# python-lz4/python-lz4

Measured on AMD Instinct MI355X. Metric: GiB/s uncompressed, device-resident, 64 KiB blocks (decompress; compress), higher is better.
Workload: dtype u8; 1 GPU; config 2: decompress 1M x 64 KiB blocks, device-resident, LZ4_compress_default input; blocks_per_gpu=1048576, block_size=65536, parallelism=shard1

## Files before the change

### python-lz4_amd/csrc/lz4m_decompress.hip

```cpp
#include "lz4m_common.h"
#include "lz4m_rows.h"
#include "lz4m_worker.h"
#include "../../include/lz4m.h"

#include <stdlib.h>
#include <string.h>

#include <atomic>
#include <mutex>

namespace lz4m {

constexpr int64_t kCoopMin = 64;

enum CopyKind : int { kNone = 0, kLiteral = 1, kMatch = 2 };

struct Copy {
    int kind;
    int64_t dpos;
    int64_t arg;
    int64_t len;
};

struct Lane {
// ... 747 lines not shown
                __builtin_amdgcn_fence(__ATOMIC_SEQ_CST, "workgroup");
                coop_copy_literal<SOLO>(d + op, s + q, lit, lane);
                __builtin_amdgcn_fence(__ATOMIC_SEQ_CST, "workgroup");
                coop_copy_match(d + opm, off, ml, lane);
                __builtin_amdgcn_fence(__ATOMIC_SEQ_CST, "workgroup");
                op = opm + ml;
                ip = qe;
                base = (op > kHistKeep ? op - kHistKeep : 0) & ~15;
                for (int32_t c = base + 16 * (int32_t)lane; c < op; c += 16 * kWave)
                    lds_st16(OB + (c - base), ld16(d + c));
                F = op;
                continue;
            }
            const bool act = (int)lane < nseq;
            const int32_t tk = act ? myseq : 0;
            const u32x4 w = HLD(IN + tk);
            const CoopSeq q = coop_parse(IN, tk, w);
            const int32_t lit = q.lit, off = q.off, ml = q.ml, adv = q.adv;
            const int32_t len = act ? lit + ml : 0;
            const int32_t o = op + wave_incl_sum(len) - len;
            const int32_t sabs = ib + myseq;
            const bool lit_ok = q.litx ? ib + q.litpos + lit <= iend - 32 && o + lit <= oend - 32
                                       : sabs + 1 <= iend - 17;
            const bool in_dict = DICT && off > o + lit && off <= o + lit + dlen && off >= 16 && o + lit - off + ml <= 0;
            const bool ok_nofit = act && q.simple && lit_ok && (!q.mlx || sabs + adv <= iend - 4) && off >= 1 &&
                                  (off <= o + lit || in_dict) && o + len < oend - 64;
            const bool ok = ok_nofit && o + len <= base + kHistW;
            const uint64_t bad = __ballot(act) & ~__ballot(ok);
            const int use = bad ? __builtin_ctzll(bad) : nseq;
            const bool fit_only = bad && ((__ballot(ok_nofit) >> use) & 1ull);
            if (use == 0 && !(fit_only && !fit_cut && op - base > kHistKeep)) break;
            fit_cut = fit_only;
            if (use == 0) continue;
            const bool u = (int)lane < use;
            const int32_t m = o + lit;
            const bool far = u && m - off < base;
            u32x4 pre = u32x4{0, 0, 0, 0};
            if (far) pre = ld16(d + (m - off) + (DICT && m - off < 0 ? ddelta : 0));
            if (u && lit > 0) {
                if (lit <= 12) {
                    HPUT(OB + (o - base), window_shift1(w), lit);
                } else {
                    for (int32_t i = 0; i < lit; i += 16)
                        HPUT(OB + (o - base + i), HLD(IN + q.litpos + i), lit - i);
                }
            }
            lds_wait();
            const int32_t src_end = m - off + (off < ml ? off : ml);
            const int32_t mend = m + ml;
            uint64_t pend = __ballot(u);
            while (pend) {
                const int32_t E = __builtin_amdgcn_readlane(m, __builtin_ctzll(pend));
                const bool mine = (pend >> lane) & 1ull;
                int32_t x = __builtin_amdgcn_update_dpp(-1, mine ? mend : -1, 0x138, 0xF, 0xF, false);
                x = max(x, __builtin_amdgcn_update_dpp(-1, x, 0x111, 0xF, 0xF, false));
                x = max(x, __builtin_amdgcn_update_dpp(-1, x, 0x112, 0xF, 0xF, false));
                x = max(x, __builtin_amdgcn_update_dpp(-1, x, 0x114, 0xF, 0xF, false));
                x = max(x, __builtin_amdgcn_update_dpp(-1, x, 0x118, 0xF, 0xF, false));
                x = max(x, __builtin_amdgcn_update_dpp(-1, x, 0x142, 0xA, 0xF, false));
                x = max(x, __builtin_amdgcn_update_dpp(-1, x, 0x143, 0xC, 0xF, false));
                const bool ready = mine && (src_end <= E || x <= m - off);
                if (ready) {
                    const int32_t s0 = m - off;
                    if (off >= 16) {
                        for (int32_t i = 0; i < ml; i += 16) {
                            const int32_t sp = s0 + i;
                            const u32x4 v = (i == 0 && far)   ? pre
                                            : sp >= base          ? HLD(OB + (sp - base))
                                                                  : ld16(d + sp + (DICT && sp < 0 ? ddelta : 0));
                            HPUT(OB + (m - base + i), v, ml - i);
                        }
                    } else {
                        const u32x4 pat = period_pattern(HLD(OB + (s0 - base)), (uint32_t)off);
                        const int32_t step = 16 - (16 % off);
                        for (int32_t i = 0; i < ml; i += step) HPUT(OB + (m - base + i), pat, ml - i);
                    }
                }
                lds_wait();
                pend &= ~__ballot(ready);
            }
            op = __builtin_amdgcn_readlane(o + len, use - 1);
            ip = ib + __builtin_amdgcn_readlane(myseq + adv, use - 1);
            for (int32_t c = F + 16 * (int32_t)lane; c + 16 <= op; c += 16 * kWave)
                st16(d + c, lds_ld16(OB + (c - base)));
            F += (op - F) & ~15;
            if (use < nseq && !fit_only) break;
        }
        if (SOLO) LZ4M_WTS(ts, 4);
        for (int32_t c = F + 16 * (int32_t)lane; c < op; c += 16 * kWave)
            gbl_put(d + c, lds_ld16(OB + (c - base)), op - c);
        __builtin_amdgcn_fence(__ATOMIC_SEQ_CST, "workgroup");
        if (SOLO) LZ4M_WTS(ts, 5);
        const int32_t r = coop_finish<DICT, SOLO>(s, d, iend, oend, ip, op, fast, lane, dlen, d + ddelta);
        if (SOLO) LZ4M_WTS(ts, 6);
        if (lane == 0) status[b] = r;
        if (SOLO && lane == 0) solo_r = r;
    }
    if constexpr (SOLO) {
        __syncthreads();
        LZ4M_WTS(ts, 2);
        const int32_t r = solo_r;
        if (solo_out != nullptr && r > 0 && solo_lit < 0) {
            const uint8_t* d0 = dst + dst_off[0];
            constexpr int32_t kStep = 16 * 256, kChunk = 16 * kStep;
            lds_u8* bounce = (lds_u8*)const_cast<uint8_t*>(solo_src);
            for (int32_t c0 = 0; c0 < r; c0 += kChunk) {
                const int32_t m = r - c0 < kChunk ? r - c0 : kChunk;
                for (int32_t base0 = 0; base0 < m; base0 += kSoloU * kStep) {
                    u32x4 v[kSoloU];
#pragma unroll
                    for (int u = 0; u < kSoloU; ++u) {
                        const int32_t p = base0 + u * kStep + 16 * (int32_t)threadIdx.x;
                        v[u] = p + 16 <= m ? ld16(d0 + c0 + p) : ld16_guarded(d0 + c0 + p, m - p);
                    }
#pragma unroll
                    for (int u = 0; u < kSoloU; ++u) {
                        const int32_t p = base0 + u * kStep + 16 * (int32_t)threadIdx.x;
                        if (p < m) lds_st16(bounce + p, v[u]);
                    }
                }
                __syncthreads();
                for (int32_t p = 16 * (int32_t)threadIdx.x; p < m; p += kStep) {
                    const u32x4 v = lds_ld16(bounce + p);
                    if (p + 16 <= m) {
                        st16(solo_out + c0 + p, v);
                    } else {
                        put_exact(solo_out + c0 + p, v, (uint32_t)(m - p));
                    }
                }
                __syncthreads();
            }
        }
        if (solo_done != nullptr) {
            __builtin_amdgcn_fence(__ATOMIC_RELEASE, "");
            __syncthreads();
            LZ4M_WTS(ts, 3);
            if (threadIdx.x == 0) __hip_atomic_store(solo_done, 1, __ATOMIC_RELEASE, __HIP_MEMORY_SCOPE_SYSTEM);
        }
    }
#undef HPUT
#undef HLD
}

template <bool DICT, bool SOLO = false>
__global__ __launch_bounds__(256, 4) void hist_decompress_kernel(const uint8_t* __restrict__ src,
                                                                 const int64_t* __restrict__ src_off,
                                                                 const int32_t* __restrict__ src_len, uint8_t* dst,
                                                                 const int64_t* __restrict__ dst_off,
                                                                 const int32_t* __restrict__ dst_cap,
                                                                 int32_t* __restrict__ status, int64_t n,
                                                                 const int32_t* __restrict__ dict_len, int64_t ddelta,
                                                                 uint8_t* solo_out, int32_t* solo_done) {
    hist_decompress_body<DICT, SOLO>(src, src_off, src_len, dst, dst_off, dst_cap, status, n, dict_len, ddelta,
                                     solo_out, solo_done);
}

__global__ __launch_bounds__(256) void decompress_worker(Mailbox* mb, uint8_t* hd, uint8_t* dbuf, uint64_t idle,
                                                        uint64_t life) {
    __shared__ uint32_t cmd[8];
    __shared__ int64_t zero_off;
    uint64_t birth = 0;
    uint32_t last = worker_init(mb, cmd, birth);
    if (threadIdx.x == 0) zero_off = 0;
    for (;;) {
        if (worker_next(mb, last, idle, birth, life, cmd) == 0) break;
        const int32_t rec_off = (int32_t)cmd[1];
        CallMeta* rec = reinterpret_cast<CallMeta*>(hd + rec_off);
        const int32_t* len_cap = reinterpret_cast<const int32_t*>(cmd + 2);
        hist_decompress_body<false, true>(hd, &zero_off, len_cap, dbuf, &zero_off, len_cap + 1, &rec->result,
                                          (int64_t)1, nullptr, (int64_t)0, hd + rec_off + kCallMeta, &rec->done);
    }
}

__device__ __forceinline__ void chain_decode(const uint8_t* __restrict__ src, const int64_t* __restrict__ src_off,
                                             const int32_t* __restrict__ src_len,
                                             const uint8_t* __restrict__ raw_flag, uint8_t* dst,
                                             int32_t* __restrict__ status, int64_t n, int32_t max_block,
                                             uint32_t lane) {
    int64_t running = 0;
    for (int64_t b = 0; b < n; ++b) {
        const int64_t len = src_len[b];
        const uint8_t* s = src + src_off[b];
        uint8_t* d = dst + running;
        if (raw_flag[b]) {
            wave_copy_wild(d, s, len, len, len, lane);
            __builtin_amdgcn_fence(__ATOMIC_SEQ_CST, "workgroup");
            if (lane == 0) status[b] = (int32_t)len;
            running += len;
            continue;
        }
        Lane L;
        L.live = false;
        L.result = -1;
        if (lane == 0) {
            L.src = s;
            L.dst = d;
            L.iend = len;
            L.oend = max_block;
            L.ip = 0;
            L.op = 0;
            L.dict_len = running < 65536 ? running : 65536;
            L.dict_end = d;
            if (L.iend <= 0) {
                L.result = -1;
            } else {
                L.fast = L.oend >= 64;
                L.live = true;
            }
        }
        while (__any(L.live)) {
            Copy lc{kNone, 0, 0, 0}, mc{kNone, 0, 0, 0};
            if (L.live) decode_step<true>(L, lc, mc);
            const uint64_t pend = __ballot(lc.kind != kNone || mc.kind != kNone);
            if (pend == 0) continue;
            __builtin_amdgcn_fence(__ATOMIC_SEQ_CST, "workgroup");
            uint8_t* dd = readlane_ptr(L.dst, 0);
            const int64_t oend = readlane64(L.oend, 0);
            if (__builtin_amdgcn_readlane(lc.kind, 0) != kNone) {
                const uint8_t* ss = readlane_ptr(L.src, 0);
                const int64_t iend = readlane64(L.iend, 0);
                const int64_t dp = readlane64(lc.dpos, 0), sp = readlane64(lc.arg, 0), ln = readlane64(lc.len, 0);
                wave_copy_wild(dd + dp, ss + sp, ln, oend - dp, iend - sp, lane);
                __builtin_amdgcn_fence(__ATOMIC_SEQ_CST, "workgroup");
            }
            if (__builtin_amdgcn_readlane(mc.kind, 0) != kNone) {
                const int64_t dp = readlane64(mc.dpos, 0), off = readlane64(mc.arg, 0), ln = readlane64(mc.len, 0);
                if (off < 0) {
                    if (lane == 0) dict_match(L, dp, -off, ln);
                } else {
                    wave_match(dd + dp, off, ln, oend - dp, lane);
                }
                __builtin_amdgcn_fence(__ATOMIC_SEQ_CST, "workgroup");
            }
        }
        const int32_t r = __builtin_amdgcn_readlane(L.result, 0);
        if (lane == 0) status[b] = r;
        if (r < 0) {
            for (int64_t k = b + 1 + lane; k < n; k += kWave) status[k] = -1;
            return;
        }
        running += r;
    }
}

__global__ __launch_bounds__(64) void decompress_chain_kernel(const uint8_t* __restrict__ src,
                                                              const int64_t* __restrict__ src_off,
                                                              const int32_t* __restrict__ src_len,
                                                              const uint8_t* __restrict__ raw_flag, uint8_t* dst,
                                                              int32_t* __restrict__ status, int64_t n,
                                                              int32_t max_block) {
    chain_decode(src, src_off, src_len, raw_flag, dst, status, n, max_block, threadIdx.x);
}

__global__ __launch_bounds__(64) void decompress_chains_kernel(const uint8_t* __restrict__ src,
                                                               const int64_t* __restrict__ src_off,
                                                               const int32_t* __restrict__ src_len,
                                                               const uint8_t* __restrict__ raw_flag,
                                                               const int64_t* __restrict__ first,
                                                               const int32_t* __restrict__ count, uint8_t* dst,
                                                               const int64_t* __restrict__ dst_off,
                                                               const int32_t* __restrict__ max_block,
                                                               int32_t* __restrict__ status) {
    const int64_t c = blockIdx.x;
    const int64_t n = count[c];
    if (n <= 0) return;
    const int64_t f = first[c];
    chain_decode(src, src_off + f, src_len + f, raw_flag + f, dst + dst_off[c], status + f, n, max_block[c],
                 threadIdx.x);
}

}

using namespace lz4m;

namespace {

int current_device() {
    int dev = 0;
    (void)hipGetDevice(&dev);
    return dev >= 0 && dev < 64 ? dev : 0;
}

constexpr int kRowsMinBlocks = 32768;

enum Decoder { kAuto = 0, kHistDec = 3, kRowsDec = 4 };

int decoder_env() {
    static const int mode = [] {
        const char* e = getenv("LZ4M_DECODER");
        if (e == nullptr) return (int)kAuto;
        if (strcmp(e, "hist") == 0) return (int)kHistDec;
        if (strcmp(e, "rows") == 0) return (int)kRowsDec;
        return (int)kAuto;
    }();
    return mode;
}

}

extern "C" size_t lz4m_decompress_workspace_bytes(void) { return 64; }

extern "C" size_t lz4m_decompress_workspace_size(int64_t n, int64_t src_bytes) {
    if (n <= 0) return 64;
    const size_t lens = (size_t)(src_bytes > 0 ? src_bytes : 0) / 3 + 17 * (size_t)n + 64;
    return (lz4m_rows_fixed_bytes(n) + lens + 255) & ~(size_t)255;
}

extern "C" int lz4m_decompress_batch_sel(const uint8_t* d_src, const int64_t* d_src_off, const int32_t* d_src_len,
                                         uint8_t* d_dst, const int64_t* d_dst_off, const int32_t* d_dst_cap,
                                         int32_t* d_status, int64_t n, void* d_work, size_t work_bytes, int decoder,
                                         lz4m_stream_t stream) {
    if (n < 0 || !(decoder == kAuto || decoder == kHistDec || decoder == kRowsDec))
        return LZ4M_EINVAL;
    if (n == 0) return 0;
    hipStream_t st = (hipStream_t)stream;
    if (decoder == kAuto) decoder = decoder_env();
    if (d_work == nullptr || work_bytes < lz4m_decompress_workspace_bytes() || ((uintptr_t)d_work & 7) != 0)
        return LZ4M_EINVAL;
    const bool rows_fit = work_bytes >= lz4m_rows_fixed_bytes(n) + 64;
    if (decoder == kAuto) decoder = rows_fit && n >= kRowsMinBlocks ? kRowsDec : kHistDec;
    if (decoder != kHistDec && !rows_fit) decoder = kHistDec;
    if (decoder == kRowsDec) {
        int pg = 1, eg = 1;
        lz4m_rows_grids(n, &pg, &eg);
        const int rc = lz4m_rows_launch(d_src, d_src_off, d_src_len, d_dst, d_dst_off, d_dst_cap, n, d_work, work_bytes,
                                        pg, eg, st);
        if (rc != 0) return rc;
        const RowMeta* meta = reinterpret_cast<const RowMeta*>(static_cast<const uint8_t*>(d_work) + kRowsMeta);
        const int64_t grid = (n + 255) / 256;
        hipLaunchKernelGGL((decompress_kernel<false, true>), dim3((uint32_t)grid), dim3(256), 0, st, d_src, d_src_off,
                           d_src_len, d_dst, d_dst_off, d_dst_cap, nullptr, nullptr, nullptr, d_status, n, meta);
        return (int)hipGetLastError();
    }
    const int64_t grid = (n + 3) / 4;
    hipLaunchKernelGGL(hist_decompress_kernel<false>, dim3((uint32_t)(grid < 65536 ? grid : 65536)), dim3(256), 0, st,
                       d_src, d_src_off, d_src_len, d_dst, d_dst_off, d_dst_cap, d_status, n, nullptr, (int64_t)0, nullptr, nullptr);
    return (int)hipGetLastError();
}

extern "C" int lz4m_decompress_solo(const uint8_t* d_src, const int64_t* d_src_off, const int32_t* d_src_len,
                                    uint8_t* d_dst, const int64_t* d_dst_off, const int32_t* d_dst_cap,
                                    int32_t* d_status, int32_t src_len_host, uint8_t* h_out, int32_t* h_done,
                                    lz4m_stream_t stream) {
    if (src_len_host < 0 || src_len_host > kSoloIn - 64) return LZ4M_EINVAL;
    hipLaunchKernelGGL((hist_decompress_kernel<false, true>), dim3(1), dim3(256), 0, (hipStream_t)stream, d_src,
                       d_src_off, d_src_len, d_dst, d_dst_off, d_dst_cap, d_status, (int64_t)1, nullptr, (int64_t)0, h_out, h_done);
    return (int)hipGetLastError();
}

extern "C" int lz4m_worker_launch(int kind, Mailbox* mb, uint8_t* hd, uint8_t* dbuf, uint64_t idle_ticks,
                                  uint64_t life_ticks, hipStream_t stream) {
    if (kind == 1) return lz4m_compress_worker_launch(mb, hd, dbuf, idle_ticks, life_ticks, stream);
    if (kind != 0) return LZ4M_EINVAL;
    hipLaunchKernelGGL(decompress_worker, dim3(1), dim3(256), 0, stream, mb, hd, dbuf, idle_ticks, life_ticks);
    return (int)hipGetLastError();
}

extern "C" int lz4m_decompress_batch_ws(const uint8_t* d_src, const int64_t* d_src_off, const int32_t* d_src_len,
                                        uint8_t* d_dst, const int64_t* d_dst_off, const int32_t* d_dst_cap,
                                        int32_t* d_status, int64_t n, void* d_work, size_t work_bytes,
                                        lz4m_stream_t stream) {
    return lz4m_decompress_batch_sel(d_src, d_src_off, d_src_len, d_dst, d_dst_off, d_dst_cap, d_status, n, d_work,
                                     work_bytes, kAuto, stream);
}

extern "C" int lz4m_decompress_batch(const uint8_t* d_src, const int64_t* d_src_off, const int32_t* d_src_len,
                                     uint8_t* d_dst, const int64_t* d_dst_off, const int32_t* d_dst_cap,
                                     int32_t* d_status, int64_t n, lz4m_stream_t stream) {
    if (n < 0) return LZ4M_EINVAL;
    if (n == 0) return 0;
    const int64_t grid = (n + 3) / 4;
    hipLaunchKernelGGL(hist_decompress_kernel<false>, dim3((uint32_t)(grid < 65536 ? grid : 65536)), dim3(256), 0,
                       (hipStream_t)stream, d_src, d_src_off, d_src_len, d_dst, d_dst_off, d_dst_cap, d_status, n,
                       nullptr, (int64_t)0, nullptr, nullptr);
    return (int)hipGetLastError();
}

extern "C" int lz4m_decompress_batch_dict(const uint8_t* d_src, const int64_t* d_src_off, const int32_t* d_src_len,
                                          uint8_t* d_dst, const int64_t* d_dst_off, const int32_t* d_dst_cap,
                                          const uint8_t* d_dict, const int64_t* d_dict_off,
                                          const int32_t* d_dict_len, int32_t* d_status, int64_t n,
                                          lz4m_stream_t stream) {
    if (n < 0) return LZ4M_EINVAL;
    if (n == 0) return 0;
    const int64_t grid = (n + 255) / 256;
    hipLaunchKernelGGL(decompress_kernel<true>, dim3((uint32_t)grid), dim3(256), 0, (hipStream_t)stream, d_src,
                       d_src_off, d_src_len, d_dst, d_dst_off, d_dst_cap, d_dict, d_dict_off, d_dict_len, d_status,
                       n, nullptr);
    return (int)hipGetLastError();
}

extern "C" int lz4m_decompress_batch_prefix(const uint8_t* d_src, const int64_t* d_src_off, const int32_t* d_src_len,
                                            uint8_t* d_dst, const int64_t* d_dst_off, const int32_t* d_dst_cap,
                                            const uint8_t* d_dict_base, const int32_t* d_dict_len,
                                            int32_t* d_status, int64_t n, lz4m_stream_t stream) {
    if (n < 0 || (n > 0 && d_dict_base == nullptr)) return LZ4M_EINVAL;
    if (n == 0) return 0;
    const int64_t grid = (n + 3) / 4;
    const int64_t delta = (int64_t)((intptr_t)d_dict_base - (intptr_t)d_dst);
    hipLaunchKernelGGL(hist_decompress_kernel<true>, dim3((uint32_t)(grid < 65536 ? grid : 65536)), dim3(256), 0,
                       (hipStream_t)stream, d_src, d_src_off, d_src_len, d_dst, d_dst_off, d_dst_cap, d_status, n,
                       d_dict_len, delta, nullptr, nullptr);
    return (int)hipGetLastError();
}

extern "C" int lz4m_decompress_chain(const uint8_t* d_src, const int64_t* d_src_off, const int32_t* d_src_len,
                                     const uint8_t* d_raw_flag, uint8_t* d_dst, int32_t* d_status, int64_t n,
                                     int32_t max_block, lz4m_stream_t stream) {
    if (n < 0 || max_block < 0) return LZ4M_EINVAL;
    if (n == 0) return 0;
    hipLaunchKernelGGL(decompress_chain_kernel, dim3(1), dim3(64), 0, (hipStream_t)stream, d_src, d_src_off,
                       d_src_len, d_raw_flag, d_dst, d_status, n, max_block);
    return (int)hipGetLastError();
}


extern "C" int lz4m_decompress_chains(const uint8_t* d_src, const int64_t* d_src_off, const int32_t* d_src_len,
                                      const uint8_t* d_raw_flag, const int64_t* d_first, const int32_t* d_count,
                                      uint8_t* d_dst, const int64_t* d_dst_off, const int32_t* d_max_block,
                                      int32_t* d_status, int64_t n_chains, lz4m_stream_t stream) {
    if (n_chains < 0 || n_chains > 0x7FFFFFFF) return LZ4M_EINVAL;
    if (n_chains == 0) return 0;
    if (!d_first || !d_count || !d_dst_off || !d_max_block || !d_status) return LZ4M_EINVAL;
    hipLaunchKernelGGL(decompress_chains_kernel, dim3((uint32_t)n_chains), dim3(64), 0, (hipStream_t)stream, d_src,
                       d_src_off, d_src_len, d_raw_flag, d_first, d_count, d_dst, d_dst_off, d_max_block, d_status);
    return (int)hipGetLastError();
}
```

### python-lz4_amd/csrc/lz4m_rows.hip

```cpp
#include "lz4m_common.h"
#include "lz4m_rows.h"

namespace lz4m {
typedef __attribute__((address_space(3))) u32x4 lds_u32x4;

__device__ __forceinline__ void wait_vm0() { __builtin_amdgcn_s_waitcnt(0x0F70); }

__device__ __forceinline__ void row_incl_sum2(int32_t& a, int32_t& b) {
    a += __builtin_amdgcn_update_dpp(0, a, 0x111, 0xF, 0xF, false);
    b += __builtin_amdgcn_update_dpp(0, b, 0x111, 0xF, 0xF, false);
    a += __builtin_amdgcn_update_dpp(0, a, 0x112, 0xF, 0xF, false);
    b += __builtin_amdgcn_update_dpp(0, b, 0x112, 0xF, 0xF, false);
    a += __builtin_amdgcn_update_dpp(0, a, 0x114, 0xF, 0xF, false);
    b += __builtin_amdgcn_update_dpp(0, b, 0x114, 0xF, 0xF, false);
    a += __builtin_amdgcn_update_dpp(0, a, 0x118, 0xF, 0xF, false);
    b += __builtin_amdgcn_update_dpp(0, b, 0x118, 0xF, 0xF, false);
}
__device__ __forceinline__ int32_t row_last(int32_t v) { return __builtin_amdgcn_update_dpp(0, v, 0x15F, 0xF, 0xF, false); }
__device__ __forceinline__ int32_t row_first(int32_t v) { return __builtin_amdgcn_update_dpp(0, v, 0x150, 0xF, 0xF, false); }

__device__ __forceinline__ void row_excl_max2(int32_t a, int32_t b, int32_t& xa, int32_t& xb) {
    int32_t x = __builtin_amdgcn_update_dpp(0, a, 0x111, 0xF, 0xF, false);
    int32_t y = __builtin_amdgcn_update_dpp(0, b, 0x111, 0xF, 0xF, false);
    x = max(x, __builtin_amdgcn_update_dpp(0, x, 0x111, 0xF, 0xF, false));
// ... 72 lines not shown

__device__ __forceinline__ int64_t whole_literal_block(const uint8_t* s, int32_t iend, int32_t oend, uint8_t* d,
                                                       uint32_t lane) {
    typedef __attribute__((address_space(1))) const uint8_t gu8;
    const int32_t y = 16 * (int32_t)lane;
    const u32x4 v = y + 16 <= iend ? ld16(s + y) : ld16_guarded(s + y, iend - y);
    const uint32_t tok = (uint32_t)__builtin_amdgcn_readlane((int32_t)v.x, 0) & 0xFFu;
    int32_t first = 16;
    for (int b = 15; b >= 0; --b)
        if (byte_of(v, b) != 255u && (lane != 0 || b != 0)) first = b;
    const uint64_t nz = __ballot(first < 16 && y + first < iend);
    if ((tok >> 4) != 15u || nz == 0) return -1;
    const int fl = __builtin_ctzll(nz);
    const int32_t pe = 16 * fl + __builtin_amdgcn_readlane(first, fl);
    const uint32_t bt = (uint32_t)__builtin_amdgcn_readlane((int32_t)byte_of(v, first & 15), fl);
    const int64_t L = 15 + 255 * (int64_t)(pe - 1) + bt;
    const int32_t q = pe + 1;
    if (q > iend - 15 || q + L != (int64_t)iend || L > oend) return -1;
    const uint8_t* cs = (const uint8_t*)(gu8*)(s + q);
    const uint32_t Lf = (uint32_t)L & ~15u;
    for (uint32_t b = 0; b < Lf; b += 4096) {
        u32x4 w[4];
#pragma unroll
        for (int u = 0; u < 4; ++u) {
            const uint32_t p = b + 1024u * u + (uint32_t)y;
            if (p < Lf) w[u] = ld16(cs + p);
        }
#pragma unroll
        for (int u = 0; u < 4; ++u) {
            const uint32_t p = b + 1024u * u + (uint32_t)y;
            if (p < Lf) st16(d + p, w[u]);
        }
    }
    if ((uint32_t)L != Lf && lane == ((Lf >> 4) & 63u)) row_put(d + Lf, ld16_guarded(cs + Lf, (int32_t)L - (int32_t)Lf), (int32_t)L - (int32_t)Lf);
    return L;
}

__global__ __launch_bounds__(kPWG) void rows_parse_kernel(const uint8_t* __restrict__ src,
                                                         const int64_t* __restrict__ src_off,
                                                         const int32_t* __restrict__ src_len,
                                                         uint8_t* __restrict__ dst,
                                                         const int64_t* __restrict__ dst_off,
                                                         const int32_t* __restrict__ dst_cap, int64_t n,
                                                         RowMeta* __restrict__ meta, uint8_t* __restrict__ lens,
                                                         int64_t lens_cap, unsigned long long* __restrict__ ctr) {
    __shared__ __attribute__((aligned(kPW))) uint8_t wins[kPWG * kPW];
    __shared__ __attribute__((aligned(kPStage))) uint8_t stgs[kPWG * kPStage];
    const uint32_t lane = lane_id();
    lds_u8* W = (lds_u8*)(wins + threadIdx.x * kPW);
    const uint32_t Wa = (uint32_t)(uintptr_t)W;
    lds_u8* stg = (lds_u8*)(stgs + threadIdx.x * kPStage);
    const uint32_t Sa = (uint32_t)(uintptr_t)stg;
    const uint8_t* s = nullptr;
    int64_t idx = -1, loff = 0;
    int32_t iend = 0, oend = 0, ip = 0, op = 0, k = 0, kf = 0, wb = 0, sh = 0;
    u32x4 pf[4];
    bool live = false, need = false, more = true, pfv = false, stall = false;
    while (true) {
        if (more) {
            const uint64_t idle = __ballot(!live);
            if (idle != 0 && (uint32_t)__popcll(idle) >= 8u) {
                const int first = __builtin_ctzll(idle);
                const uint32_t cnt = (uint32_t)__popcll(idle);
                unsigned long long qb = 0;
                if ((int)lane == first) qb = atomicAdd(&ctr[0], (unsigned long long)cnt);
                qb = (unsigned long long)readlane64((int64_t)qb, first);
                if (qb + cnt >= (unsigned long long)n) more = false;
                int64_t wantb = 0;
                bool fresh = false;
                if (!live) {
                    const uint64_t below = lane == 0 ? 0 : (idle & (~0ull >> (64 - lane)));
                    idx = (int64_t)(qb + (unsigned long long)__popcll(below));
                    if (idx < n) {
                        const int64_t so = src_off[idx];
                        const int32_t il = src_len[idx];
                        sh = (int32_t)((uintptr_t)(src + so) & 63u);
                        if (so < sh) sh = 0;
                        s = src + so - sh;
                        iend = il + sh;
                        oend = dst_cap[idx];
                        ip = sh;
                        op = k = kf = 0;
                        wb = -4 * kPW;
                        pfv = false;
                        if (oend >= 64 && il > 0) {
                            const int32_t a = il / 3, b = oend / 4;
                            wantb = ((int64_t)(a < b ? a : b) + 1 + 15) & ~(int64_t)15;
                            fresh = true;
                        } else {
                            meta[idx] = RowMeta{0, 0, 0, 0, 0, 0};
                        }
                    }
                }
                int64_t incl = wantb;
#pragma unroll
                for (int dd = 1; dd < 64; dd <<= 1) {
                    const int64_t t = __shfl_up(incl, dd);
                    if ((int)lane >= dd) incl += t;
                }
                const int64_t total = readlane64(incl, 63);
                int64_t abase = 0;
                if (total > 0) {
                    if (lane == 0) abase = (int64_t)atomicAdd(&ctr[1], (unsigned long long)total);
                    abase = readlane64(abase, 0);
                }
                if (fresh) {
                    loff = abase + incl - wantb;
                    if (loff + wantb > lens_cap) {
                        meta[idx] = RowMeta{0, 0, 0, 0, 0, 0};
                    } else {
                        live = true;
                        need = true;
                    }
                }
            }
        }
        if (!__any(live)) {
            if (more) continue;
            break;
        }
        {
            const uint64_t R = __ballot(live && pfv && ip >= wb + 64);
            if (R) {
#pragma unroll
                for (int c = 0; c < 4; ++c) {
                    const int bb = 16 * c + (int)(lane >> 2);
                    const int32_t wbb = __builtin_amdgcn_ds_bpermute(bb << 2, wb);
                    if ((R >> bb) & 1ull) {
                        lds_u8* Wb = (lds_u8*)(wins + bb * kPW);
                        const int32_t h = (wbb >> 6) & 1;
                        lds_st16(Wb + 64 * h + 16 * (int32_t)(lane & 3), pf[c]);
                    }
                }
                if ((R >> lane) & 1ull) {
                    wb += 64;
                    pfv = false;
                }
            }
        }
        if (live && stall && !need && ip + 16 > wb + kPW) need = true;
        stall = false;
        bool wl = false;
        if (live && need) {
            need = false;
            if (ip + 32 > wb + kPW) {
                const int32_t nb = ip & ~63;
                u32x4 v0[4], v1[4];
                load64(s, nb, iend, v0);
                load64(s, nb + 64, iend, v1);
                ring_put(W, (nb >> 6) & 1, v0);
                ring_put(W, ((nb >> 6) + 1) & 1, v1);
                wb = nb;
                pfv = false;
            }
            bool good = true, slow = true;
            int32_t pe = 0;
            int64_t lit = 0, ml = 0;
            {
                const uint32_t x0 = __builtin_amdgcn_alignbyte(*(lds_vu32*)(size_t)(Wa | (((uint32_t)ip + 4u) & (kPW - 4))),
                                                               *(lds_vu32*)(size_t)(Wa | ((uint32_t)ip & (kPW - 4))), (uint32_t)ip);
                const uint32_t tok = x0 & 0xFFu;
                const int32_t l0 = (int32_t)(tok >> 4), mlc = (int32_t)(tok & 15u);
                int32_t q = 1, L = l0;
                bool g = true, sl = false;
                if (l0 == 15) {
                    if (ip + 1 >= iend - 15) {
                        g = false;
                    } else {
                        const int32_t e = (int32_t)((x0 >> 8) & 0xFFu);
                        q = 2;
                        L += e;
                        if (ip + 2 > iend - 15) g = false;
                        else if (e == 255) sl = true;
                        if (g && !sl && (op + L > oend - 32 || ip + q + L > iend - 32)) g = false;
                    }
                } else if (ip + 1 > iend - 17) {
                    g = false;
                }
                int32_t M = mlc, pq = 0;
                if (g && !sl) {
                    const int32_t po = q + L;
                    if (po + 3 > 32) {
                        sl = true;
                    } else {
                        const uint32_t ao = (uint32_t)(ip + po);
                        const uint32_t dw = __builtin_amdgcn_alignbyte(*(lds_vu32*)(size_t)(Wa | ((ao + 4u) & (kPW - 4))),
                                                                       *(lds_vu32*)(size_t)(Wa | (ao & (kPW - 4))), ao);
                        const int32_t off = (int32_t)(dw & 0xFFFFu);
                        pq = po + 2;
                        if (mlc == 15) {
                            const int32_t e2 = (int32_t)((dw >> 16) & 0xFFu);
                            ++pq;
                            M += e2;
                            if (ip + pq > iend - 4) g = false;
                            else if (e2 == 255) sl = true;
                        }
                        M += 4;
                        if (g && !sl && (off == 0 || off > op + L || op + L + M >= oend - 64)) g = false;
                    }
                }
                slow = sl;
                if (!sl) {
                    good = g;
                    pe = ip + pq;
                    lit = L;
                    ml = M;
                }
            }
            if (slow) {
#define PB(x) ((x) - wb < kPW ? (uint32_t)W[(x) & (kPW - 1)] : (uint32_t)s[(x)])
                good = true;
                const uint32_t tok = PB(ip);
                lit = tok >> 4;
                int32_t q = ip + 1;
                if (lit == 15) {
                    if (q >= iend - 15) {
                        good = false;
                    } else {
                        uint32_t b;
                        int32_t run = 0;
                        do {
                            b = PB(q);
                            ++q;
                            lit += b;
                            if (q > iend - 15) good = false;
                            if (++run >= kPRunCap && b == 255) {
                                good = false;
                                wl = k == 0;
                            }
                        } while (good && b == 255);
                        if (good && (op + lit > oend - 32 || q + lit > iend - 32)) good = false;
                    }
                } else if (q > iend - 17) {
                    good = false;
                }
                if (good) {
                    const int32_t po = q + (int32_t)lit;
                    const uint32_t off = PB(po) | (PB(po + 1) << 8);
                    pe = po + 2;
                    ml = tok & 15;
                    if (ml == 15) {
                        uint32_t b;
                        int32_t run = 0;
                        do {
                            b = PB(pe);
                            ++pe;
                            ml += b;
                            if (pe > iend - 4) good = false;
                            if (++run >= kPRunCap && b == 255) good = false;
                        } while (good && b == 255);
                    }
                    ml += 4;
                    if (good && (off == 0 || (int64_t)off > (int64_t)op + lit || (int64_t)op + lit + ml >= (int64_t)oend - 64))
                        good = false;
                }
#undef PB
            }
            if (good) {
                const int32_t adv = pe - ip;
                stg[k & (kPStage - 1)] = (uint8_t)(adv < 255 ? adv : 255);
                ip = pe;
                op += (int32_t)(lit + ml);
                ++k;
            } else {
                for (int32_t c = kf; c < k; c += 16) row_put(lens + loff + c, lds_ld16(stg + (c & (kPStage - 1))), k - c);
                meta[idx] = RowMeta{loff, k, ip - sh, op, 0, 0};
                live = false;
            }
        }
        for (uint64_t C = __ballot(wl); C != 0; C &= C - 1) {
            const int f = __builtin_ctzll(C);
            const int64_t fi = readlane64(idx, f);
            const int32_t fsh = __builtin_amdgcn_readlane(sh, f);
            const int64_t r = whole_literal_block(readlane_ptr(s, f) + fsh, __builtin_amdgcn_readlane(iend, f) - fsh,
                                                  __builtin_amdgcn_readlane(oend, f), dst + dst_off[fi], lane);
            if ((int)lane == f && r >= 0) meta[idx] = RowMeta{loff, 0, kRowsWholeLiteral, (int32_t)r, 0, 0};
        }
        if (live && k - kf >= kPStage / 2) {
            uint8_t* o = lens + loff + kf;
            st16(o, lds_ld16(stg + (kf & (kPStage - 1))));
            kf += kPStage / 2;
        }
        {
            const uint64_t Q = __ballot(live && !pfv && wb + kPW < iend);
            if (Q) {
                const uint64_t na = (uint64_t)(uintptr_t)(s + wb + kPW);
                const int32_t left = iend - (wb + kPW);
#pragma unroll
                for (int c = 0; c < 4; ++c) {
                    const int bb = 16 * c + (int)(lane >> 2);
                    const uint32_t lo = (uint32_t)__builtin_amdgcn_ds_bpermute(bb << 2, (int32_t)(uint32_t)na);
                    const uint32_t hi = (uint32_t)__builtin_amdgcn_ds_bpermute(bb << 2, (int32_t)(uint32_t)(na >> 32));
                    const int32_t lf = __builtin_amdgcn_ds_bpermute(bb << 2, left) - 16 * (int32_t)(lane & 3);
                    if ((Q >> bb) & 1ull) {
                        const uint8_t* q = readlane_safe_ptr(((uint64_t)hi << 32) | lo) + 16 * (lane & 3);
                        pf[c] = lf >= 16 ? ld16(q) : ld16_guarded(q, lf);
                    }
                }
                if ((Q >> lane) & 1ull) pfv = true;
            }
        }
        const int32_t thr = min(kPMinActive, (int)__popcll(__ballot(live)));
        const int32_t kfl = kf + kPStage - 1;
        auto peek = [&](int32_t& lit, int32_t& adv, int32_t& ml, int32_t& off, int32_t& oe) __attribute__((always_inline)) {
            const int32_t tok = (int32_t)*(lds_vu8*)(size_t)(Wa | ((uint32_t)ip & (kPW - 1)));
            lit = tok >> 4;
            const int32_t mlc = tok & 15;
            const int32_t ob = ip + 1 + lit;
            const uint32_t lo = *(lds_vu32*)(size_t)(Wa | ((uint32_t)ob & (kPW - 4)));
            const uint32_t hi = *(lds_vu32*)(size_t)(Wa | ((uint32_t)(ob + 4) & (kPW - 4)));
            const uint32_t dw = __builtin_amdgcn_alignbyte(hi, lo, (uint32_t)ob);
            const bool mlx = mlc == 15;
            off = (int32_t)(dw & 0xFFFFu);
            adv = 3 + lit + (int32_t)mlx;
            ml = mlc + 4 + (mlx ? (int32_t)((dw >> 16) & 0xFFu) : 0);
            oe = op + lit + ml;
        };
        {
            const int32_t lim = min(wb + kPW - 16, iend - 20);
            const int32_t oendm = oend - 64;
            bool go = live && !need && !stall;
            while (true) {
#pragma unroll
                for (int u = 0; u < kPSteps; ++u) {
                    int32_t lit, adv, ml, off, oe;
                    peek(lit, adv, ml, off, oe);
                    const bool take = go & (ip <= lim) & (k < kfl) & (lit <= 12) & (ml != 274) &
                                      ((uint32_t)(off - 1) < (uint32_t)(op + lit)) & (oe < oendm);
                    *(lds_vu8*)(size_t)(Sa | ((uint32_t)k & (kPStage - 1))) = (uint8_t)adv;
                    ip += take ? adv : 0;
                    op = take ? oe : op;
                    k += (int32_t)take;
                    go = take;
                }
                if ((int)__popcll(__ballot(go)) < max(thr, 1)) break;
            }
            if (live && !need && !stall && !go) {
                int32_t lit, adv, ml, off, oe;
                peek(lit, adv, ml, off, oe);
                const bool fast = (lit <= 12) & (ml != 274) & (ip <= iend - 20) & (off != 0) & (off <= op + lit) &
                                  (oe < oendm);
                stall = true;
                need = (ip + 16 <= wb + kPW) & (k < kfl) & !fast;
            }
        }
    }
}

constexpr int32_t kRowsH = 1280;
constexpr int32_t kRowsHS = kRowsH + 32;
constexpr int32_t kRowsRoom = 512;
constexpr int32_t kRowsKeep = kRowsH - kRowsRoom;
static_assert(kRowsKeep % 16 == 0 && kRowsKeep + kRowsRoom <= kRowsH && kRowsKeep + 16 <= 1024, "history split");

__device__ __forceinline__ void row_copy_literal(uint8_t* d, const uint8_t* s, int32_t len, int32_t jj) {
    for (int32_t pos = 16 * jj; pos < len; pos += 256) {
        const u32x4 v = len - pos >= 16 ? ld16(s + pos) : ld16_guarded(s + pos, len - pos);
        row_put(d + pos, v, len - pos);
    }
}

__device__ __forceinline__ void row_copy_match(uint8_t* d, int32_t off, int32_t len, int32_t jj) {
    if (off >= 16) {
        const int32_t w = off & ~15;
        for (int32_t b = 0; b < len; b += w) {
            const int32_t e = min(b + w, len);
            for (int32_t p0 = b + 16 * jj; p0 < e; p0 += 1024) {
                u32x4 v[4];
#pragma unroll
                for (int u = 0; u < 4; ++u)
                    if (p0 + 256 * u < e) v[u] = ld16(d + p0 + 256 * u - off);
#pragma unroll
                for (int u = 0; u < 4; ++u)
                    if (p0 + 256 * u < e) row_put(d + p0 + 256 * u, v[u], len - (p0 + 256 * u));
            }
            __builtin_amdgcn_fence(__ATOMIC_SEQ_CST, "workgroup");
        }
        return;
    }
    const u32x4 pat = period_pattern(ld16(d - off), (uint32_t)off);
    const int32_t step = 16 - (16 % off);
    for (int32_t pos = step * jj; pos < len; pos += step * 16) row_put(d + pos, pat, len - pos);
}


#define LDS_PUT(p, v, k) lds_put_al((p), (v), (k), MT)

#define ROFF(x) ((uint32_t)(x))

struct PSeq {
    int32_t t, lit, off, ml, o, dlt;
    int32_t opn, ipn;
    uint32_t fl;
};
constexpr uint32_t kFlU = 1, kFlFar = 2, kFlLate = 4, kFlLitHbm = 8, kFlEsc = 16;

struct FarSrc {
    u32x4 g0, g1;
};

__device__ __forceinline__ void parse_round(PSeq& P, int32_t jj, int32_t r, int32_t k0, int32_t nseq, int32_t ip,
                                            int32_t op, int32_t bnext, int32_t F, const uint8_t* s, const uint8_t* d,
                                            int32_t iend, int32_t dlt, int32_t t, u32x4 wa, u32x4 wb, lds_u32x4* XS,
                                            FarSrc& FS, int32_t& incsum) {
    const bool act = k0 + jj < nseq;
    const bool esc = dlt == 255;
    const bool wbok = t + 32 <= iend;
    const uint32_t tok = wa.x & 0xFFu;
    const int32_t lit0 = (int32_t)(tok >> 4);
    const bool litx = lit0 == 15;
    const int32_t lit = lit0 + (litx ? (int32_t)byte_of(wa, 1) : 0);
    const int32_t lp = litx ? 2 : 1;
    const int32_t po = lp + lit;
    const int32_t mlc = (int32_t)(tok & 15u);
    const uint32_t pq = (uint32_t)(po < 28 ? po : 28);
    const uint32_t dwo = dword32_tree(wa, wb, pq);
    const uint32_t bsh = po > 28 ? 8u : 0u;
    int32_t off = (int32_t)((dwo >> bsh) & 0xFFFFu);
    const int32_t e0 = (int32_t)((dwo >> (bsh + 16)) & 0xFFu);
    int32_t ml = mlc + (mlc == 15 ? e0 : 0);
    const bool slow = (po + 3 > 32) | ((mlc == 15) & (e0 == 255)) | ((po + 3 > 16) & !wbok);
    if (slow && act && !esc) {
        const uint8_t* q = s + t;
        off = (int32_t)q[po] | ((int32_t)q[po + 1] << 8);
        ml = mlc;
        if (ml == 15) {
            int32_t pe = po + 2;
            uint32_t b;
            do {
                b = q[pe];
                ++pe;
                ml += (int32_t)b;
            } while (b == 255 && pe < iend - t);
        }
    }
    ml += 4;
    const int32_t len = act && !esc ? lit + ml : 0;
    int32_t lsum = len;
    row_incl_sum2(lsum, incsum);
    const int32_t o = op + lsum - len;
    const int32_t mend = o + lit + ml;
    const bool ok = act & !esc & (mend <= bnext + kRowsH);
    const uint64_t nok = __ballot(!ok);
    int32_t use;
    bool u;
    if (nok == 0) {
        use = 16;
        u = true;
        P.opn = row_last(o + len);
        P.ipn = row_last(t + dlt);
    } else {
        const uint32_t rb = (uint32_t)(nok >> (16 * r)) & 0xFFFFu;
        use = rb ? __builtin_ctz(rb) : 16;
        u = jj < use;
        P.opn = op + row_last(row_incl_sum(u ? len : 0));
        P.ipn = ip + row_last(row_incl_sum(u ? dlt : 0));
    }
    const int32_t s0 = o + lit - off;
    const bool far = u & (s0 < bnext);
    const bool late = far & (s0 + 32 > F);
    const bool pf = far & !late;
    FS.g0 = ld16(d + ROFF(pf ? s0 : 0));
    FS.g1 = ld16(d + ROFF((pf & (ml > 16)) ? s0 + 16 : 0));
    const uint32_t sh = (uint32_t)lp;
    XS[0] = u32x4{__builtin_amdgcn_alignbyte(wa.y, wa.x, sh), __builtin_amdgcn_alignbyte(wa.z, wa.y, sh),
                 __builtin_amdgcn_alignbyte(wa.w, wa.z, sh), __builtin_amdgcn_alignbyte(wb.x, wa.w, sh)};
    XS[1] = u32x4{__builtin_amdgcn_alignbyte(wb.y, wb.x, sh), __builtin_amdgcn_alignbyte(wb.z, wb.y, sh),
                 __builtin_amdgcn_alignbyte(wb.w, wb.z, sh), __builtin_amdgcn_alignbyte(0u, wb.w, sh)};
    P.t = t + lp;
    P.lit = lit;
    P.off = off;
    P.ml = ml;
    P.o = o;
    P.dlt = dlt;
    P.fl = ((uint32_t)use << 8) | (u ? kFlU : 0u) | (far ? kFlFar : 0u) | (late ? kFlLate : 0u) | (esc ? kFlEsc : 0u) |
           ((u & (lp + lit > 16) & ((lp + lit > 32) | !wbok)) ? kFlLitHbm : 0u);
}

__device__ __forceinline__ int32_t cold_j16(int32_t jj) {
    int32_t v = 16 * jj;
    asm volatile("" : "+v"(v));
    return v;
}

__device__ __forceinline__ int32_t next_base(int32_t op, int32_t base) {
    return op - base > kRowsH - kRowsRoom ? ((op - kRowsKeep) & ~15) : base;
}

__device__ __forceinline__ void load_in(const uint8_t* s, int32_t t, int32_t iend, u32x4& a, u32x4& b) {
    const int32_t ta = t + 16 <= iend ? t : 0;
    const int32_t tb = t + 32 <= iend ? t + 16 : iend - 16;
    a = ld16(s + ROFF(ta));
    b = ld16(s + ROFF(tb));
}
__device__ __forceinline__ int32_t load_len(const uint8_t* dl, int32_t k, int32_t nseq) {
    return (int32_t)dl[ROFF(k < nseq ? k : nseq - 1)];
}


constexpr int kEWG = 256;
__global__ __launch_bounds__(kEWG) __attribute__((amdgpu_waves_per_eu(5, 8))) void rows_exec_kernel(const uint8_t* __restrict__ src,
                                                       const int64_t* __restrict__ src_off,
                                                       const int32_t* __restrict__ src_len, uint8_t* dst,
                                                       const int64_t* __restrict__ dst_off,
                                                       const RowMeta* __restrict__ meta,
                                                       const uint8_t* __restrict__ lens, int64_t n,
                                                       unsigned long long* __restrict__ ctr) {
    __shared__ __attribute__((aligned(16))) uint8_t hists[kEWG / 16 * kRowsHS];
    __shared__ __attribute__((aligned(16))) uint32_t mtab[kPutTab];
    __shared__ __attribute__((aligned(16))) uint32_t psel[16 * 8];
    __shared__ __attribute__((aligned(16))) u32x4 xsl[kEWG * 2];
    const uint32_t lane = threadIdx.x & 63u;
    const int32_t jj = (int32_t)(lane & 15), r = (int32_t)(lane >> 4);
    lds_u8* HB = (lds_u8*)(hists + (threadIdx.x >> 4) * kRowsHS);
    lds_put_table_init(mtab, threadIdx.x, kEWG);
    lds_cu32* MT = (lds_cu32*)mtab;
    period_sel_init(psel, threadIdx.x, kEWG);
    __syncthreads();
    lds_cu32* PS = (lds_cu32*)psel;
    lds_u32x4* XSL = (lds_u32x4*)(xsl + 2 * threadIdx.x);
    const uint8_t* s = nullptr;
    uint8_t* d = nullptr;
    const uint8_t* dl = nullptr;
    int32_t iend = 0, nseq = 0, k0 = 0, ip = 0, op = 0, base = 0, F = 0;
    bool have = false, sync = true;
    PSeq P, Q;
    FarSrc FS;
    int32_t incq = 0, lraw = 0;
    u32x4 na = u32x4{0, 0, 0, 0}, nb = na;
    while (true) {
        if (!have) {
            unsigned long long b = 0;
            if (jj == 0) b = atomicAdd(&ctr[2], 1ull);
            const uint32_t blo = (uint32_t)row_first((int32_t)(uint32_t)b);
            const uint32_t bhi = (uint32_t)row_first((int32_t)(uint32_t)(b >> 32));
            b = ((unsigned long long)bhi << 32) | blo;
            if (b >= (unsigned long long)n) break;
            const RowMeta mt = meta[b];
            if (mt.nseq == 0) continue;
            s = src + src_off[b];
            d = dst + dst_off[b];
            iend = src_len[b];
            dl = lens + mt.loff;
            nseq = mt.nseq;
            k0 = ip = op = base = F = 0;
            have = true;
            sync = true;
        }
        if (sync && k0 >= nseq) {
            for (int32_t c = F + cold_j16(jj); c < op; c += 256) row_put(d + c, lds_ld16(HB + (c - base)), op - c);
            have = false;
            continue;
        }
        if (sync) {
            const int32_t dc = load_len(dl, k0 + jj, nseq);
            const int32_t dq = load_len(dl, k0 + 16 + jj, nseq);
            lraw = load_len(dl, k0 + 32 + jj, nseq);
            int32_t incc = dc;
            incq = dq;
            row_incl_sum2(incc, incq);
            const int32_t tc = ip + incc - dc;
            u32x4 wa, wb;
            load_in(s, tc, iend, wa, wb);
            load_in(s, ip + row_last(incc) + incq - dq, iend, na, nb);
            int32_t dummy = 0;
            parse_round(P, jj, r, k0, nseq, ip, op, base, F, s, d, iend, dc, tc, wa, wb, XSL, FS, dummy);
            sync = false;
            if ((P.fl >> 8) != 0) wait_vm0();
        }
        if ((P.fl >> 8) == 0) {
            sync = true;
            int32_t L, q, ofs, qe, M;
            if (!(row_first((int32_t)P.fl) & kFlEsc)) {
                L = row_first(P.lit);
                q = row_first(P.t);
                ofs = row_first(P.off);
                M = row_first(P.ml);
                qe = q + L + 2 + (M >= 19 ? (M - 19) / 255 + 1 : 0);
            } else {
                const uint32_t tk = s[ip];
                L = (int32_t)(tk >> 4);
                q = ip + 1;
                if (L == 15) {
                    uint32_t b;
                    do {
                        b = s[q];
                        ++q;
                        L += (int32_t)b;
                    } while (b == 255 && q < iend);
                }
                ofs = (int32_t)s[q + L] | ((int32_t)s[q + L + 1] << 8);
                qe = q + L + 2;
                M = (int32_t)(tk & 15u);
                if (M == 15) {
                    uint32_t b;
                    do {
                        b = s[qe];
                        ++qe;
                        M += (int32_t)b;
                    } while (b == 255 && qe < iend);
                }
                M += 4;
            }
            for (int32_t c = F + cold_j16(jj); c < op; c += 256) row_put(d + c, lds_ld16(HB + (c - base)), op - c);
            row_copy_literal(d + op, s + q, L, jj);
            __builtin_amdgcn_fence(__ATOMIC_SEQ_CST, "workgroup");
            row_copy_match(d + op + L, ofs, M, jj);
            __builtin_amdgcn_fence(__ATOMIC_SEQ_CST, "workgroup");
            op += L + M;
            ip = qe;
            k0 += 1;
            base = (op > kRowsKeep ? op - kRowsKeep : 0) & ~15;
            for (int32_t c = base + cold_j16(jj); c < op; c += 256) lds_st16(HB + (c - base), ld16(d + c));
            F = op;
            continue;
        }
        {
            const bool u = (P.fl & kFlU) != 0;
            const int32_t lit = P.lit, o = P.o;
            if (u && lit > 0) LDS_PUT(HB + (o - base), XSL[0], lit);
            if (u && lit > 16) {
                if (!(P.fl & kFlLitHbm)) {
                    LDS_PUT(HB + (o - base + 16), XSL[1], lit - 16);
                } else {
                    for (int32_t i = 16; i < lit; i += 16) LDS_PUT(HB + (o - base + i), ld16(s + P.t + i), lit - i);
                }
            }
        }
        const bool ahead = (P.fl >> 8) == 16 && k0 + 16 < nseq;
        auto parse_ahead = [&]() __attribute__((always_inline)) {
            if (ahead) {
                const int32_t bq = next_base(P.opn, base);
                const int32_t dq = incq - __builtin_amdgcn_update_dpp(0, incq, 0x111, 0xF, 0xF, true);
                int32_t inc2 = lraw;
                parse_round(Q, jj, r, k0 + 16, nseq, P.ipn, P.opn, bq, F, s, d, iend, dq, P.ipn + incq - dq, na, nb, XSL, FS, inc2);
                incq = inc2;
                load_in(s, Q.ipn + incq - lraw, iend, na, nb);
                lraw = load_len(dl, k0 + 48 + jj, nseq);
            }
        };
        const bool u = (P.fl & kFlU) != 0;
        const int32_t lit = P.lit, off = P.off, ml = P.ml, o = P.o;
        const int32_t m = o + lit, mend = m + ml, s0 = m - off;
        const bool far = (P.fl & kFlFar) != 0, late = (P.fl & kFlLate) != 0;
        u32x4 g0 = FS.g0;
        const u32x4 g1 = FS.g1;
        if (__any(late)) {
            const u32x4 lv = ld16(d + ROFF(late ? s0 : 0));
            g0 = late ? lv : g0;
        }
        const int32_t se = s0 + (off < ml ? off : ml);
        const bool per = off < 16;
        constexpr uint64_t kRem16 = (0ull << 3) | (0ull << 6) | (1ull << 9) | (0ull << 12) | (1ull << 15) |
                                    (4ull << 18) | (2ull << 21) | (0ull << 24) | (7ull << 27) | (6ull << 30) |
                                    (5ull << 33) | (4ull << 36) | (3ull << 39) | (2ull << 42) | (1ull << 45);
        const int32_t stp = per ? 16 - (int32_t)((kRem16 >> (3u * ((uint32_t)off & 15u))) & 7u) : 16;
        bool pend = u;
        auto copy_match = [&]() __attribute__((always_inline)) {
            const u32x4 l0 = lds_ld16a(HB + (s0 >= base ? s0 - base : 0));
            u32x4 v0 = far ? g0 : l0;
            if (per) v0 = period_perm(l0, PS + 8 * off);
            LDS_PUT(HB + (m - base), v0, ml);
            if (ml > stp) {
                for (int32_t i = stp; i < ml; i += stp) {
                    u32x4 v = v0;
                    if (!per) {
                        const int32_t sp = s0 + i;
                        v = lds_ld16a(HB + (sp >= base ? sp - base : 0));
                        const bool pc1 = (i == 16) & far & !late;
                        if (sp < base && pc1) v = g1;
                        const bool hb = (sp < base) & !pc1;
                        if (__any(hb)) {
                            const u32x4 x = ld16(d + ROFF(hb ? sp : 0));
                            v = hb ? x : v;
                        }
                    }
                    LDS_PUT(HB + (m - base + i), v, ml - i);
                }
            }
        };
        while (__any(pend)) {
            int32_t x1, y1;
            row_excl_max2(pend ? mend + 1 : 0, pend ? 0x3FFFFFFF - m : 0, x1, y1);
            const bool ready = pend & ((x1 <= s0 + 1) | (y1 <= 0x3FFFFFFF - se));
            if (ready) copy_match();
            pend = pend && !ready;
        }
        parse_ahead();
        const int32_t opn = P.opn;
        {
            const int32_t fe = opn & ~127;
            for (int32_t c = F + 16 * jj; c + 16 <= fe; c += 256) st16(d + ROFF(c), lds_ld16(HB + (c - base)));
            if (fe > F) F += (fe - F) & ~15;
        }
        op = opn;
        ip = P.ipn;
        k0 += (int32_t)(P.fl >> 8);
        const int32_t nbse = next_base(op, base);
        if (nbse != base) {
            for (int32_t c0 = 0; c0 < op - nbse; c0 += 1024) {
                u32x4 v[4];
#pragma unroll
                for (int g = 0; g < 4; ++g) v[g] = lds_ld16(HB + (nbse - base) + c0 + 256 * g + 16 * jj);
#pragma unroll
                for (int g = 0; g < 4; ++g) lds_st16(HB + c0 + 256 * g + 16 * jj, v[g]);
            }
            base = nbse;
        }
        if (ahead) {
            P = Q;
        } else {
            sync = true;
        }
    }
}

}

using namespace lz4m;


extern "C" size_t lz4m_rows_fixed_bytes(int64_t n) { return kRowsMeta + (size_t)n * sizeof(RowMeta); }

extern "C" int lz4m_rows_launch(const uint8_t* d_src, const int64_t* d_src_off, const int32_t* d_src_len,
                                uint8_t* d_dst, const int64_t* d_dst_off, const int32_t* d_dst_cap, int64_t n,
                                void* d_work, size_t work_bytes, int parse_grid, int exec_grid, hipStream_t stream) {
    const size_t fixed = lz4m_rows_fixed_bytes(n);
    if (work_bytes < fixed) return LZ4M_ROWS_ENOSPACE;
    unsigned long long* ctr = static_cast<unsigned long long*>(d_work);
    RowMeta* meta = reinterpret_cast<RowMeta*>(static_cast<uint8_t*>(d_work) + kRowsMeta);
    uint8_t* lens = static_cast<uint8_t*>(d_work) + fixed;
    const int64_t lens_cap = (int64_t)(work_bytes - fixed);
    hipError_t e = hipMemsetAsync(ctr, 0, 64, stream);
    if (e != hipSuccess) return (int)e;
    hipLaunchKernelGGL(rows_parse_kernel, dim3((uint32_t)parse_grid), dim3(kPWG), 0, stream, d_src, d_src_off,
                       d_src_len, d_dst, d_dst_off, d_dst_cap, n, meta, lens, lens_cap, ctr);
    hipLaunchKernelGGL(rows_exec_kernel, dim3((uint32_t)exec_grid), dim3(kEWG), 0, stream, d_src, d_src_off, d_src_len,
                       d_dst, d_dst_off, meta, lens, n, ctr);
    return (int)hipGetLastError();
}

extern "C" int lz4m_rows_grids(int64_t n, int* parse_grid, int* exec_grid) {
    int dev = 0, cus = 0, pk = 0, ek = 0;
    (void)hipGetDevice(&dev);
    (void)hipDeviceGetAttribute(&cus, hipDeviceAttributeMultiprocessorCount, dev);
    (void)hipOccupancyMaxActiveBlocksPerMultiprocessor(&pk, reinterpret_cast<const void*>(rows_parse_kernel), kPWG, 0);
    (void)hipOccupancyMaxActiveBlocksPerMultiprocessor(&ek, reinterpret_cast<const void*>(rows_exec_kernel), kEWG, 0);
    if (cus <= 0) cus = 256;
    const int64_t ps = (int64_t)cus * (pk > 0 ? pk : 1), es = (int64_t)cus * (ek > 0 ? ek : 1);
    const int64_t pneed = (n + kPWG - 1) / kPWG, eneed = (n + kEWG / 16 - 1) / (kEWG / 16);
    *parse_grid = (int)(pneed < ps ? pneed : ps);
    *exec_grid = (int)(eneed < es ? eneed : es);
    return 0;
}
```

Baseline: 584.0 GiB/s.

## Carry next LZ4 token in registers, restripe literal slots, align lens buffer

The parse kernel's fast loop now takes the next token byte from the dword it already reads for the offset, so each step skips one LDS byte load. The kfl bound check moves out of the unrolled steps to once per iteration. The exec kernel's per-thread literal staging slots are restriped from two adjacent entries per thread to stride-256 planes, which is meant to cut LDS bank conflicts. The lens buffer is also padded to 16-byte alignment, with the workspace size grown to fit. The hoisted kfl guard can stop the unrolled batch slightly early near the stage limit.

```diff
diff --git a/python-lz4_amd/csrc/lz4m_decompress.hip b/python-lz4_amd/csrc/lz4m_decompress.hip
--- a/python-lz4_amd/csrc/lz4m_decompress.hip
+++ b/python-lz4_amd/csrc/lz4m_decompress.hip
@@ -1073,7 +1073,7 @@
 
 extern "C" size_t lz4m_decompress_workspace_size(int64_t n, int64_t src_bytes) {
     if (n <= 0) return 64;
-    const size_t lens = (size_t)(src_bytes > 0 ? src_bytes : 0) / 3 + 17 * (size_t)n + 64;
+    const size_t lens = (size_t)(src_bytes > 0 ? src_bytes : 0) / 3 + 17 * (size_t)n + 64 + 16;
     return (lz4m_rows_fixed_bytes(n) + lens + 255) & ~(size_t)255;
 }
 
diff --git a/python-lz4_amd/csrc/lz4m_rows.hip b/python-lz4_amd/csrc/lz4m_rows.hip
--- a/python-lz4_amd/csrc/lz4m_rows.hip
+++ b/python-lz4_amd/csrc/lz4m_rows.hip
@@ -398,8 +398,8 @@
         }
         const int32_t thr = min(kPMinActive, (int)__popcll(__ballot(live)));
         const int32_t kfl = kf + kPStage - 1;
-        auto peek = [&](int32_t& lit, int32_t& adv, int32_t& ml, int32_t& off, int32_t& oe) __attribute__((always_inline)) {
-            const int32_t tok = (int32_t)*(lds_vu8*)(size_t)(Wa | ((uint32_t)ip & (kPW - 1)));
+        auto peek = [&](int32_t tok, int32_t& lit, int32_t& adv, int32_t& ml, int32_t& off, int32_t& oe,
+                        int32_t& ntok) __attribute__((always_inline)) {
             lit = tok >> 4;
             const int32_t mlc = tok & 15;
             const int32_t ob = ip + 1 + lit;
@@ -411,29 +411,34 @@
             adv = 3 + lit + (int32_t)mlx;
             ml = mlc + 4 + (mlx ? (int32_t)((dw >> 16) & 0xFFu) : 0);
             oe = op + lit + ml;
+            ntok = (int32_t)(mlx ? dw >> 24 : (dw >> 16) & 0xFFu);
         };
         {
             const int32_t lim = min(wb + kPW - 16, iend - 20);
             const int32_t oendm = oend - 64;
             bool go = live && !need && !stall;
+            int32_t tok = (int32_t)*(lds_vu8*)(size_t)(Wa | ((uint32_t)ip & (kPW - 1)));
             while (true) {
+                go &= k <= kfl - kPSteps;
 #pragma unroll
                 for (int u = 0; u < kPSteps; ++u) {
-                    int32_t lit, adv, ml, off, oe;
-                    peek(lit, adv, ml, off, oe);
-                    const bool take = go & (ip <= lim) & (k < kfl) & (lit <= 12) & (ml != 274) &
+                    int32_t lit, adv, ml, off, oe, ntok;
+                    peek(tok, lit, adv, ml, off, oe, ntok);
+                    const bool take = go & (ip <= lim) & (lit <= 12) & (ml != 274) &
                                       ((uint32_t)(off - 1) < (uint32_t)(op + lit)) & (oe < oendm);
                     *(lds_vu8*)(size_t)(Sa | ((uint32_t)k & (kPStage - 1))) = (uint8_t)adv;
                     ip += take ? adv : 0;
                     op = take ? oe : op;
                     k += (int32_t)take;
+                    tok = ntok;
                     go = take;
                 }
                 if ((int)__popcll(__ballot(go)) < max(thr, 1)) break;
             }
             if (live && !need && !stall && !go) {
-                int32_t lit, adv, ml, off, oe;
-                peek(lit, adv, ml, off, oe);
+                int32_t lit, adv, ml, off, oe, ntok;
+                tok = (int32_t)*(lds_vu8*)(size_t)(Wa | ((uint32_t)ip & (kPW - 1)));
+                peek(tok, lit, adv, ml, off, oe, ntok);
                 const bool fast = (lit <= 12) & (ml != 274) & (ip <= iend - 20) & (off != 0) & (off <= op + lit) &
                                   (oe < oendm);
                 stall = true;
@@ -448,6 +453,7 @@
 constexpr int32_t kRowsRoom = 512;
 constexpr int32_t kRowsKeep = kRowsH - kRowsRoom;
 static_assert(kRowsKeep % 16 == 0 && kRowsKeep + kRowsRoom <= kRowsH && kRowsKeep + 16 <= 1024, "history split");
+constexpr int32_t kRowsOver = kRowsRoom + 1024 - kRowsHS;
 
 __device__ __forceinline__ void row_copy_literal(uint8_t* d, const uint8_t* s, int32_t len, int32_t jj) {
     for (int32_t pos = 16 * jj; pos < len; pos += 256) {
@@ -484,6 +490,7 @@
 
 #define ROFF(x) ((uint32_t)(x))
 
+constexpr int kXsStride = 256;
 struct PSeq {
     int32_t t, lit, off, ml, o, dlt;
     int32_t opn, ipn;
@@ -561,7 +568,7 @@
     const uint32_t sh = (uint32_t)lp;
     XS[0] = u32x4{__builtin_amdgcn_alignbyte(wa.y, wa.x, sh), __builtin_amdgcn_alignbyte(wa.z, wa.y, sh),
                  __builtin_amdgcn_alignbyte(wa.w, wa.z, sh), __builtin_amdgcn_alignbyte(wb.x, wa.w, sh)};
-    XS[1] = u32x4{__builtin_amdgcn_alignbyte(wb.y, wb.x, sh), __builtin_amdgcn_alignbyte(wb.z, wb.y, sh),
+    XS[kXsStride] = u32x4{__builtin_amdgcn_alignbyte(wb.y, wb.x, sh), __builtin_amdgcn_alignbyte(wb.z, wb.y, sh),
                  __builtin_amdgcn_alignbyte(wb.w, wb.z, sh), __builtin_amdgcn_alignbyte(0u, wb.w, sh)};
     P.t = t + lp;
     P.lit = lit;
@@ -595,6 +602,7 @@
 
 
 constexpr int kEWG = 256;
+static_assert(kXsStride == kEWG, "the literal slots: one entry per thread, twice");
 __global__ __launch_bounds__(kEWG) __attribute__((amdgpu_waves_per_eu(5, 8))) void rows_exec_kernel(const uint8_t* __restrict__ src,
                                                        const int64_t* __restrict__ src_off,
                                                        const int32_t* __restrict__ src_len, uint8_t* dst,
@@ -614,7 +622,7 @@
     period_sel_init(psel, threadIdx.x, kEWG);
     __syncthreads();
     lds_cu32* PS = (lds_cu32*)psel;
-    lds_u32x4* XSL = (lds_u32x4*)(xsl + 2 * threadIdx.x);
+    lds_u32x4* XSL = (lds_u32x4*)(xsl + threadIdx.x);
     const uint8_t* s = nullptr;
     uint8_t* d = nullptr;
     const uint8_t* dl = nullptr;
@@ -717,7 +725,7 @@
             if (u && lit > 0) LDS_PUT(HB + (o - base), XSL[0], lit);
             if (u && lit > 16) {
                 if (!(P.fl & kFlLitHbm)) {
-                    LDS_PUT(HB + (o - base + 16), XSL[1], lit - 16);
+                    LDS_PUT(HB + (o - base + 16), XSL[kXsStride], lit - 16);
                 } else {
                     for (int32_t i = 16; i < lit; i += 16) LDS_PUT(HB + (o - base + i), ld16(s + P.t + i), lit - i);
                 }
@@ -801,6 +809,7 @@
 #pragma unroll
                 for (int g = 0; g < 4; ++g) lds_st16(HB + c0 + 256 * g + 16 * jj, v[g]);
             }
+            static_assert(kRowsOver > 0 && kRowsOver < 256, "the rebase copy's reads past a row's slot");
             base = nbse;
         }
         if (ahead) {
@@ -825,8 +834,9 @@
     if (work_bytes < fixed) return LZ4M_ROWS_ENOSPACE;
     unsigned long long* ctr = static_cast<unsigned long long*>(d_work);
     RowMeta* meta = reinterpret_cast<RowMeta*>(static_cast<uint8_t*>(d_work) + kRowsMeta);
-    uint8_t* lens = static_cast<uint8_t*>(d_work) + fixed;
-    const int64_t lens_cap = (int64_t)(work_bytes - fixed);
+    const size_t pad = (size_t)((0 - (reinterpret_cast<uintptr_t>(d_work) + fixed)) & 15u);
+    uint8_t* lens = static_cast<uint8_t*>(d_work) + fixed + pad;
+    const int64_t lens_cap = work_bytes - fixed > pad ? (int64_t)(work_bytes - fixed - pad) : 0;
     hipError_t e = hipMemsetAsync(ctr, 0, 64, stream);
     if (e != hipSuccess) return (int)e;
     hipLaunchKernelGGL(rows_parse_kernel, dim3((uint32_t)parse_grid), dim3(kPWG), 0, stream, d_src, d_src_off,
```

After: 587.9 GiB/s, median of 6. Within noise of the previous version (+0.7%).
